# burn-research/OpenMEASURE

Hardware: AMD Instinct MI355X
Metric: SPR fit+reconstruct throughput (GB/s snapshot matrix) (higher is better)
Workload: dtype f64

## Files before the change

### openmeasure_amd/csrc/common.hpp

```cpp
#pragma once
#include <hip/hip_runtime.h>
#include <stdint.h>
#include <stdio.h>

#include "spr_hip.h"

typedef double f64x4 __attribute__((ext_vector_type(4)));
typedef double f64x2 __attribute__((ext_vector_type(2)));

void spr_set_error(const char *fmt, ...);

#define SPR_REQUIRE(cond, code, ...)      \
  do {                                    \
    if (!(cond)) {                        \
      spr_set_error(__VA_ARGS__);         \
      return (code);                      \
    }                                     \
  } while (0)

#define SPR_HIP_TRY(expr)                                                          \
  do {                                                                             \
    hipError_t e__ = (expr);                                                       \
    if (e__ != hipSuccess) {                                                       \
      spr_set_error("%s failed: %s (%s:%d)", #expr, hipGetErrorString(e__),       \
                    __FILE__, __LINE__);                                           \
      return SPR_E_HIP;                                                            \
    }                                                                              \
  } while (0)

#define SPR_LAUNCH_CHECK()                                                         \
  do {                                                                             \
    hipError_t e__ = hipGetLastError();                                            \
    if (e__ != hipSuccess) {                                                       \
      spr_set_error("kernel launch failed: %s (%s:%d)", hipGetErrorString(e__),   \
                    __FILE__, __LINE__);                                           \
      return SPR_E_HIP;                                                            \
    }                                                                              \
  } while (0)

int spr_cached_cus();

struct SegPlan {
  int64_t row0, n_rows, n_points;
  int32_t n_features;
  int32_t total_wg;
  int32_t chunk_rows;
};

__host__ __device__ inline void seg_range(const SegPlan &p, int f, int64_t &lo, int64_t &hi) {
  int64_t glo = (int64_t)f * p.n_points, ghi = glo + p.n_points;
  if (glo < p.row0) glo = p.row0;
  if (ghi > p.row0 + p.n_rows) ghi = p.row0 + p.n_rows;
  if (ghi < glo) ghi = glo;
  lo = glo - p.row0;
  hi = ghi - p.row0;
}

__host__ __device__ inline int seg_wgs(const SegPlan &p, int64_t rows) {
  if (rows <= 0) return 0;
  int64_t w = rows * (int64_t)p.total_wg / p.n_rows;
  int64_t chunks = (rows + p.chunk_rows - 1) / p.chunk_rows;
  if (w > chunks) w = chunks;
  if (w < 1) w = 1;
  return (int)w;
}

__host__ __device__ inline int seg_first_feature(const SegPlan &p) { return (int)(p.row0 / p.n_points); }
__host__ __device__ inline int seg_last_feature(const SegPlan &p) {
  int64_t f = (p.row0 + p.n_rows - 1) / p.n_points;
// ... 7 lines not shown
    int64_t lo, hi;
    seg_range(p, f, lo, hi);
    tot += seg_wgs(p, hi - lo);
  }
  return tot;
}

__device__ inline bool seg_locate(const SegPlan &p, int b, int &f, int &wl, int &wpf, int &base,
                                  int64_t &lo, int64_t &hi) {
  int acc = 0;
  int f1 = seg_last_feature(p);
  for (int ff = seg_first_feature(p); ff <= f1; ++ff) {
    seg_range(p, ff, lo, hi);
    int w = seg_wgs(p, hi - lo);
    if (b < acc + w) {
      f = ff; wl = b - acc; wpf = w; base = acc;
      return true;
    }
    acc += w;
  }
  return false;
}

template <int CTRL>
__device__ inline double dpp_f64(double v) {
  union { double d; int i[2]; } a, b;
  a.d = v;
  b.i[0] = __builtin_amdgcn_update_dpp(0, a.i[0], CTRL, 0xF, 0xF, true);
  b.i[1] = __builtin_amdgcn_update_dpp(0, a.i[1], CTRL, 0xF, 0xF, true);
  return b.d;
}

template <int WIDTH>
__device__ inline double group_sum_t(double v) {
  if (WIDTH >= 2) v += dpp_f64<0xB1>(v);
  if (WIDTH >= 4) v += dpp_f64<0x4E>(v);
  if (WIDTH >= 8) v += dpp_f64<0x141>(v);
  if (WIDTH >= 16) v += dpp_f64<0x140>(v);
  if (WIDTH >= 32) v += __shfl_xor(v, 16, 64);
  if (WIDTH >= 64) v += __shfl_xor(v, 32, 64);
  return v;
}

__device__ inline double group_sum(double v, int width) {
  for (int o = width >> 1; o > 0; o >>= 1) v += __shfl_xor(v, o, 64);
  return v;
// ... 16 lines not shown
```

### openmeasure_amd/csrc/project_ws.hip

```cpp
#include <type_traits>

#include "rowtile.hpp"

namespace {

#ifndef WS_ABLATE
#define WS_ABLATE 0
#endif
constexpr int WS_WAVES = 8;
constexpr int WS_ROWS = 16 * WS_WAVES;

template <int RT> struct WsLds { static constexpr int NC = 16 * RT, LDW = NC; static_assert(RT % 2 == 0, "column tiles come in pairs"); };

template <typename TX> struct WsPiece;
template <> struct WsPiece<double> { f64x2 a, b; };
template <> struct WsPiece<float> { float x, y, z, w; };

template <int VEC, typename TX>
__device__ inline WsPiece<TX> ws_load(const TX *__restrict__ rp, int col0, int m) {
  WsPiece<TX> p;
  if constexpr (std::is_same<TX, double>::value) {
    if (VEC) {
      p.a = *reinterpret_cast<const f64x2 *>(rp + col0);
      p.b = *reinterpret_cast<const f64x2 *>(rp + col0 + 2);
// ... 8 lines not shown
    } else {
      p.x = rp[col0 < m ? col0 : 0];         p.y = rp[col0 + 1 < m ? col0 + 1 : 0];
      p.z = rp[col0 + 2 < m ? col0 + 2 : 0]; p.w = rp[col0 + 3 < m ? col0 + 3 : 0];
    }
  }
  return p;
}

template <typename TX>
__device__ inline double ws_elem(const WsPiece<TX> &p, int t) {
  if constexpr (std::is_same<TX, double>::value) return t == 0 ? p.a.x : t == 1 ? p.a.y : t == 2 ? p.b.x : p.b.y;
  else return (double)(t == 0 ? p.x : t == 1 ? p.y : t == 2 ? p.z : p.w);
}

template <int MT, int RT, int VEC, typename TX, typename TU, bool NRM>
__global__ __launch_bounds__(WS_WAVES * 64) void project_ws_kernel(
    const TX *__restrict__ X, int64_t ldx, int m, int center_i, SegPlan plan, const double *__restrict__ inv_scale,
    const double *__restrict__ rowmean, const double *__restrict__ W, int r, TU *__restrict__ Ur, int64_t ldu,
    double *__restrict__ nrm2) {
  constexpr int K = 16 * MT, NJ = MT;
  constexpr int NC = WsLds<RT>::NC, LDW = WsLds<RT>::LDW;
  __shared__ double Wl[K * LDW];

  int f, wl, wpf, base;
  int64_t lo, hi;
  if (!seg_locate(plan, blockIdx.x, f, wl, wpf, base, lo, hi)) return;

  const int lane = threadIdx.x & 63;
  const int wave = __builtin_amdgcn_readfirstlane(threadIdx.x >> 6);
  const int li = lane & 15, kk = lane >> 4;
  const double isc = inv_scale[f];

  for (int e = threadIdx.x; e < K * NC; e += WS_WAVES * 64) {
    const int k = e / NC, c = e - k * NC;
    Wl[k * LDW + (c >> 5) * 32 + (c & 15) * 2 + ((c >> 4) & 1)] = (k < m && c < r) ? W[(int64_t)k * r + c] * isc : 0.0;
  }
  __syncthreads();
  double wbar[RT];
#pragma unroll
  for (int ct = 0; ct < RT; ++ct) {
    double sacc = 0.0;
    if (center_i != 0) {
      for (int k = kk; k < K; k += 4) sacc += Wl[k * LDW + (ct >> 1) * 32 + li * 2 + (ct & 1)];
      sacc += __shfl_xor(sacc, 16, 64);
      sacc += __shfl_xor(sacc, 32, 64);
    }
    wbar[ct] = sacc;
  }

  const int64_t nchunks = (hi - lo + WS_ROWS - 1) / WS_ROWS;
  int64_t c = wl;
  if (c >= nchunks) return;
  const double *wb = Wl + (4 * kk) * LDW + 2 * li;
  const double *wb_hi = wb + 128 * LDW;

  auto row_ptr = [&](int64_t cc) {
    int64_t row = lo + cc * WS_ROWS + 16 * wave + li;
    row = row < hi ? row : hi - 1;
    return X + row * ldx;
  };
  WsPiece<TX> areg[NJ];
  {
    const TX *rp = row_ptr(c);
#pragma unroll
    for (int j = 0; j < NJ; ++j) areg[j] = ws_load<VEC, TX>(rp, 16 * j + 4 * kk, m);
  }
  while (c < nchunks) {
    const int64_t cn = c + wpf;
    const TX *rpn = row_ptr(cn < nchunks ? cn : c);
    const int64_t blk0 = lo + c * WS_ROWS + 16 * wave;
    double mu[4];
#pragma unroll
    for (int i = 0; i < 4; ++i) {
      const int64_t rr = blk0 + kk + 4 * i;
      const double v = rowmean[rr < hi ? rr : hi - 1];
      mu[i] = center_i != 0 ? v : 0.0;
    }
    f64x4 acc[RT];
#pragma unroll
    for (int ct = 0; ct < RT; ++ct) acc[ct] = (f64x4){0.0, 0.0, 0.0, 0.0};
    f64x2 bcur[RT / 2], bnxt[RT / 2];
#pragma unroll
    for (int p = 0; p < RT / 2; ++p) bcur[p] = *reinterpret_cast<const f64x2 *>(wb + 32 * p);
#pragma unroll
    for (int j = 0; j < NJ; ++j) {
#pragma unroll
      for (int t = 0; t < 4; ++t) {
        const int sn = 4 * j + t + 1;
        const int jn = (sn >> 2) % NJ, tn = sn & 3;
        const double *wj = (jn < 8 ? wb : wb_hi) + (16 * (jn & 7) + tn) * LDW;
#pragma unroll
        for (int p = 0; p < RT / 2; ++p) bnxt[p] = *reinterpret_cast<const f64x2 *>(wj + 32 * p);
        const double a = ws_elem<TX>(areg[j], t);
#pragma unroll
        for (int p = 0; p < RT / 2; ++p) {
#if WS_ABLATE == 1
          asm volatile("" ::"v"(a), "v"(bcur[p].x), "v"(bcur[p].y));
#else
          acc[2 * p] = __builtin_amdgcn_mfma_f64_16x16x4f64(a, bcur[p].x, acc[2 * p], 0, 0, 0);
          acc[2 * p + 1] = __builtin_amdgcn_mfma_f64_16x16x4f64(a, bcur[p].y, acc[2 * p + 1], 0, 0, 0);
#endif
        }
        if (t == 3) areg[j] = ws_load<VEC, TX>(rpn, 16 * j + 4 * kk, m);
        __builtin_amdgcn_sched_group_barrier(0x100, RT / 2, 0);
        __builtin_amdgcn_sched_group_barrier(0x008, RT, 0);
        __builtin_amdgcn_sched_barrier(0);
#pragma unroll
        for (int p = 0; p < RT / 2; ++p) bcur[p] = bnxt[p];
      }
    }
    {
      const bool full = (blk0 + 16 <= hi) && (r == NC);
      TU *up = Ur + (blk0 + kk) * ldu + li;
      double q[4] = {0.0, 0.0, 0.0, 0.0};
#pragma unroll
      for (int ct = 0; ct < RT; ++ct) {
        const double s[4] = {acc[ct].x - mu[0] * wbar[ct], acc[ct].y - mu[1] * wbar[ct],
                             acc[ct].z - mu[2] * wbar[ct], acc[ct].w - mu[3] * wbar[ct]};
        if (NRM) {
#pragma unroll
          for (int i = 0; i < 4; ++i) { const double v = (double)(TU)s[i]; q[i] = fma(v, v, q[i]); }
        }
        if (full) {
#pragma unroll
          for (int i = 0; i < 4; ++i) up[4 * i * ldu + 16 * ct] = (TU)s[i];
        } else if (16 * ct + li < r) {
#pragma unroll
          for (int i = 0; i < 4; ++i)
            if (blk0 + kk + 4 * i < hi) up[4 * i * ldu + 16 * ct] = (TU)s[i];
        }
      }
      if (NRM) {
#pragma unroll
        for (int i = 0; i < 4; ++i) {
          const double t = group_sum_t<16>(q[i]);
          if (li == i && blk0 + kk + 4 * i < hi) nrm2[blk0 + kk + 4 * i] = t;
        }
      }
    }
    c = cn;
  }
}

template <int MT, int RT, typename TX, typename TU>
int ws_launch(const TX *X, int64_t n_rows, int32_t m, int64_t ldx, int64_t row0, int64_t n_points, int32_t n_features,
              int center, const double *inv_scale, const double *rowmean, const double *W, int32_t r, TU *Ur,
              int64_t ldu, int accumulate, double *nrm2, hipStream_t st) {
  const int cus = spr_cached_cus();
  SegPlan plan;
  plan.row0 = row0; plan.n_rows = n_rows; plan.n_points = n_points; plan.n_features = n_features;
  static const int narrow_per_cu = [] { const char *e = getenv("SPR_WS_WG_PER_CU"); const int v = e ? atoi(e) : 2; return v >= 1 && v <= 4 ? v : 2; }();
  plan.total_wg = (cus > 0 ? cus : 256) * (MT <= 4 ? narrow_per_cu : 1);
  plan.chunk_rows = WS_ROWS;
  const int grid = seg_total_wgs(plan);
  const bool vec = (m == 16 * MT) && ((sizeof(TX) * ldx) % 16 == 0) && ((reinterpret_cast<uintptr_t>(X) & 15) == 0);
  if (!vec) return SPR_E_UNSUPPORTED;
  if (nrm2)
    hipLaunchKernelGGL((project_ws_kernel<MT, RT, 1, TX, TU, true>), dim3(grid), dim3(WS_WAVES * 64), 0, st, X, ldx, (int)m,
                       center, plan, inv_scale, rowmean, W, (int)r, Ur, ldu, nrm2);
  else
    hipLaunchKernelGGL((project_ws_kernel<MT, RT, 1, TX, TU, false>), dim3(grid), dim3(WS_WAVES * 64), 0, st, X, ldx, (int)m,
                       center, plan, inv_scale, rowmean, W, (int)r, Ur, ldu, nrm2);
  SPR_LAUNCH_CHECK();
  return SPR_OK;
}

}

#include "project_ws.hpp"

template <typename TX, typename TU>
int spr_project_ws(const TX *d_X, int64_t n_rows, int32_t m, int64_t ldx, int64_t row0, int64_t n_points,
                   int32_t n_features, int32_t center, const double *d_inv_scale, const double *d_rowmean,
                   const double *d_W, int32_t r, TU *d_Ur, int64_t ldu, int32_t accumulate, double *d_rownorm2,
                   hipStream_t st) {
  if (accumulate) return SPR_E_UNSUPPORTED;
  const int mt = spr_round_mt(m);
// ... 27 lines not shown
```

### openmeasure_amd/csrc/runtime.hip

```cpp
#include <stdarg.h>
#include <stdlib.h>
#include <string.h>

#include "common.hpp"

namespace {
thread_local char g_err[512] = "";
}

void spr_set_error(const char *fmt, ...) {
  va_list ap;
  va_start(ap, fmt);
  vsnprintf(g_err, sizeof(g_err), fmt, ap);
  va_end(ap);
}

int spr_cached_cus() {
  static int cus = 0;
  if (cus) return cus;
  int dev = 0;
  hipDeviceProp_t prop;
  if (hipGetDevice(&dev) != hipSuccess || hipGetDeviceProperties(&prop, dev) != hipSuccess) return 0;
  cus = prop.multiProcessorCount;
  if (const char *e = getenv("SPR_RESERVE_CUS")) {
    const int k = atoi(e);
    if (k > 0 && k < cus) cus -= k;
  }
  return cus;
}

extern "C" int spr_abi_version(void) { return SPR_ABI_VERSION; }

extern "C" const char *spr_last_error(void) { return g_err; }

extern "C" int spr_device_cus(int *out_cus) {
  SPR_REQUIRE(out_cus != nullptr, SPR_E_INVALID, "spr_device_cus: NULL output");
  const int c = spr_cached_cus();
  SPR_REQUIRE(c > 0, SPR_E_HIP, "spr_device_cus: no HIP device");
  *out_cus = c;
  return SPR_OK;
}

namespace {
__global__ __launch_bounds__(256) void upload_kernel(const uint64_t *__restrict__ src, uint64_t *__restrict__ dst,
                                                     int64_t n_words) {
  for (int64_t i = (int64_t)blockIdx.x * 256 + threadIdx.x; i < n_words; i += (int64_t)gridDim.x * 256)
    dst[i] = __builtin_nontemporal_load(src + i);
}
}

extern "C" int spr_upload_bytes(void *d_dst, const void *h_pinned_src, int64_t n_bytes, void *stream) {
// ... 38 lines not shown
```

### openmeasure_amd/csrc/stats_gram.hip

```cpp
#include <stdlib.h>

#include <type_traits>

#include "rowtile.hpp"

#ifndef GRAM_UNIT_PAIRING
#define GRAM_UNIT_PAIRING 1
#endif
#ifndef GRAM_ABLATE
#define GRAM_ABLATE 0
#endif
#if GRAM_ABLATE == 1
#define GRAM_MFMA(a, b, c) ({ asm volatile("" ::"v"(a), "v"(b)); (c); })
#else
#define GRAM_MFMA(a, b, c) __builtin_amdgcn_mfma_f64_16x16x4f64((a), (b), (c), 0, 0, 0)
#endif

namespace {

template <int MT>
struct GramShape {
  static constexpr int MPAD = 16 * MT;
  static constexpr int MP = MPAD + ((MT % 2 == 0) ? 16 : 0);
  static constexpr int T = MT * (MT + 1) / 2;
// ... 11 lines not shown
template <> struct GramCfg<4>  { static constexpr int NW = 8,  R = GRAM4_R, KS = 4; static constexpr bool DBUF = true; static constexpr int LPRMAX = GRAM4_LPR; };
template <> struct GramCfg<6>  { static constexpr int NW = 12, R = 48, KS = 4; static constexpr bool DBUF = true; static constexpr int LPRMAX = 16; };
template <> struct GramCfg<8>  { static constexpr int NW = 8,  R = 32, KS = 2; static constexpr bool DBUF = true; static constexpr int LPRMAX = 16; };
template <> struct GramCfg<12> { static constexpr int NW = 12, R = 24, KS = 2; static constexpr bool DBUF = false; static constexpr int LPRMAX = 32; };
#ifndef GRAM_DBUF16
#define GRAM_DBUF16 false
#endif
template <> struct GramCfg<16> { static constexpr int NW = 8,  R = 32, KS = 1; static constexpr bool DBUF = GRAM_DBUF16; static constexpr int LPRMAX = 16; };

template <int MT> struct GramOut { static constexpr int KSO = (GramCfg<MT>::KS >= 4) ? 1 : GramCfg<MT>::KS; };

constexpr int tri_index(int mt, int ti, int tj) { return ti * mt - ti * (ti - 1) / 2 + (tj - ti); }

template <int MT>
__device__ inline void tile_coords(int idx, int &ti, int &tj) {
  ti = 0;
  while (ti < MT - 1 && idx >= MT - ti) { idx -= MT - ti; ++ti; }
  tj = ti + idx;
  if (tj > MT - 1) tj = MT - 1;
}

template <int MT, int U, int VEC, typename TX>
__device__ inline void gram_wave(const TX *__restrict__ X, int64_t ldx, int m, int center,
                                 int64_t lo, int64_t hi, int wl, int wpf, int ks, int wave, int lane,
                                 double *__restrict__ lds0, double *__restrict__ lds1,
                                 double *__restrict__ rowmean, double *__restrict__ stat_part,
                                 double *__restrict__ slab, double *__restrict__ rowsum) {
  using S = GramShape<MT>;
  using C = GramCfg<MT>;
  constexpr int R = C::R, KS = C::KS, NW = C::NW, MP = S::MP, T = S::T;
  constexpr int KROWS = R / KS, KSTEPS = KROWS / 4;
  constexpr int RA = U, RB = MT - 1 - U;
  constexpr int NA = MT - RA;
  constexpr int NB = (RB != RA) ? MT - RB : 0;
  static_assert(KROWS % 4 == 0, "k slice must be a multiple of the MFMA depth");
  using RT = RowTile<MT, R, MP, NW, C::LPRMAX, TX>;

  f64x4 accA[NA];
  f64x4 accB[NB > 0 ? NB : 1];
#pragma unroll
  for (int j = 0; j < NA; ++j) accA[j] = (f64x4){0.0, 0.0, 0.0, 0.0};
#pragma unroll
  for (int j = 0; j < NB; ++j) accB[j] = (f64x4){0.0, 0.0, 0.0, 0.0};

  RowStats st;
  st.init();
  RT tile;
// ... 80 lines not shown
        }
#pragma unroll
        for (int j = 0; j < NB; ++j) {
          double *tp = red + tri_index(MT, RB, RB + j) * 256;
          tp[0] = accB[j].x; tp[64] = accB[j].y; tp[128] = accB[j].z; tp[192] = accB[j].w;
        }
      }
      __syncthreads();
      if (ks == s - 1) {
#pragma unroll
        for (int j = 0; j < NA; ++j) {
          const double *tp = red + tri_index(MT, RA, RA + j) * 256;
          accA[j].x += tp[0]; accA[j].y += tp[64]; accA[j].z += tp[128]; accA[j].w += tp[192];
        }
#pragma unroll
        for (int j = 0; j < NB; ++j) {
          const double *tp = red + tri_index(MT, RB, RB + j) * 256;
          accB[j].x += tp[0]; accB[j].y += tp[64]; accB[j].z += tp[128]; accB[j].w += tp[192];
        }
      }
    }
  }
  if (KSO == KS || ks == 0) {
    double *sp = slab + ((int64_t)blockIdx.x * KSO + (KSO == KS ? ks : 0)) * T * 256 + lane;
#pragma unroll
    for (int j = 0; j < NA; ++j) {
      double *tp = sp + (int64_t)tri_index(MT, RA, RA + j) * 256;
      tp[0] = accA[j].x; tp[64] = accA[j].y; tp[128] = accA[j].z; tp[192] = accA[j].w;
    }
#pragma unroll
    for (int j = 0; j < NB; ++j) {
      double *tp = sp + (int64_t)tri_index(MT, RB, RB + j) * 256;
      tp[0] = accB[j].x; tp[64] = accB[j].y; tp[128] = accB[j].z; tp[192] = accB[j].w;
    }
  }
  if ((lane % RT::LPR) == 0) {
    double *q = stat_part + ((int64_t)blockIdx.x * RT::ROWS_PER_IT + wave * RT::RPW + lane / RT::LPR) * 3;
    q[0] = st.cnt; q[1] = st.mean(); q[2] = st.m2();
  }
}

__device__ inline void chan_merge(double &n, double &mu, double &m2, double nb, double mb, double sb) {
  if (nb > 0.0) {
    const double tot = n + nb, d = mb - mu;
    mu += d * nb / tot;
    m2 += sb + d * d * n * nb / tot;
    n = tot;
  }
}

template <int MT, int U, typename TX, bool EXT, bool SUMS>
__device__ inline void gram_wave_own(const TX *__restrict__ X, int64_t ldx, int64_t lo, int64_t hi, int wl, int wpf, int ks,
                                     int wave, int lane, double *__restrict__ lds0, double *__restrict__ lds1,
                                     double *__restrict__ rowmean, double *__restrict__ slab, double *__restrict__ rowsum) {
  using S = GramShape<MT>;
  using C = GramCfg<MT>;
  constexpr int R = C::R, KS = C::KS, NW = C::NW, MP = S::MP, T = S::T;
  constexpr int KROWS = R / KS, KSTEPS = KROWS / 4;
  constexpr int RA = U, RB = MT - 1 - U;
  constexpr int NA = MT - RA;
  constexpr int NB = (RB != RA) ? MT - RB : 0;
  using RT = RowTile<MT, R, MP, NW, C::LPRMAX, TX>;

  f64x4 accA[NA];
  f64x4 accB[NB > 0 ? NB : 1];
#pragma unroll
  for (int j = 0; j < NA; ++j) accA[j] = (f64x4){0.0, 0.0, 0.0, 0.0};
#pragma unroll
  for (int j = 0; j < NB; ++j) accB[j] = (f64x4){0.0, 0.0, 0.0, 0.0};

  RT tile;
  const int64_t nchunks = (hi - lo + R - 1) / R;
  const int64_t lane_off = (int64_t)(wave * RT::RPW + lane / RT::LPR) * ldx;
  auto base_of = [&](int64_t row0) { return X + row0 * ldx; };
  int64_t c = wl;
// ... 45 lines not shown
        for (int j = 0; j < NA; ++j) accA[j] = GRAM_MFMA(op[k & 1][0], op[k & 1][j], accA[j]);
#pragma unroll
        for (int j = 0; j < NB; ++j) accB[j] = GRAM_MFMA(op[k & 1][RB - RA], op[k & 1][RB - RA + j], accB[j]);
        if (nfull) stage(std::true_type{}, k); else stage(std::false_type{}, k);
      }
    } else {
#pragma unroll
      for (int k = 0; k < KSTEPS; ++k) {
        double op[NA];
#pragma unroll
        for (int j = 0; j < NA; ++j) op[j] = p[k * 4 * MP + 16 * j];
#pragma unroll
        for (int j = 0; j < NA; ++j) accA[j] = GRAM_MFMA(op[0], op[j], accA[j]);
#pragma unroll
        for (int j = 0; j < NB; ++j) accB[j] = GRAM_MFMA(op[RB - RA], op[RB - RA + j], accB[j]);
        if (nfull) stage(std::true_type{}, k); else stage(std::false_type{}, k);
      }
    }
    buf ^= 1;
    c = cn;
    cn = c2;
    nrow0 = n2row0;
  }
  double *sp = slab + ((int64_t)blockIdx.x * KS + ks) * T * 256 + lane;
#pragma unroll
  for (int j = 0; j < NA; ++j) {
    double *tp = sp + (int64_t)tri_index(MT, RA, RA + j) * 256;
    tp[0] = accA[j].x; tp[64] = accA[j].y; tp[128] = accA[j].z; tp[192] = accA[j].w;
  }
#pragma unroll
  for (int j = 0; j < NB; ++j) {
    double *tp = sp + (int64_t)tri_index(MT, RB, RB + j) * 256;
    tp[0] = accB[j].x; tp[64] = accB[j].y; tp[128] = accB[j].z; tp[192] = accB[j].w;
  }
}

template <int MT, typename TX, bool EXT, bool SUMS>
__global__ __launch_bounds__(GramCfg<MT>::NW * 64) void stats_gram_own_kernel(
    const TX *__restrict__ X, int64_t ldx, SegPlan plan, double *__restrict__ rowmean, double *__restrict__ slab,
    double *__restrict__ rowsum) {
  using S = GramShape<MT>;
  using C = GramCfg<MT>;
  constexpr int NU = S::NU;
  __shared__ double lds[2][C::R * S::MP];
  int f, wl, wpf, base;
  int64_t lo, hi;
  if (!seg_locate(plan, blockIdx.x, f, wl, wpf, base, lo, hi)) return;
  const int lane = threadIdx.x & 63;
  const int wave = __builtin_amdgcn_readfirstlane(threadIdx.x >> 6);
  const int ks = wave / NU;
  const int unit = (GRAM_UNIT_PAIRING && NU == 8 && C::KS == 1) ? ((wave < 4) ? wave : 11 - wave) : wave % NU;
#define GRAM_UNIT(UV)                                                                                          \
  case UV:                                                                                                     \
    if constexpr (UV < NU)                                                                                     \
      gram_wave_own<MT, UV, TX, EXT, SUMS>(X, ldx, lo, hi, wl, wpf, ks, wave, lane, lds[0], lds[1], rowmean, slab, rowsum); \
    break;
  switch (unit) {
    GRAM_UNIT(0) GRAM_UNIT(1) GRAM_UNIT(2) GRAM_UNIT(3) GRAM_UNIT(4) GRAM_UNIT(5) GRAM_UNIT(6) GRAM_UNIT(7)
    default: break;
  }
#undef GRAM_UNIT
}

constexpr int RS_THREADS = 1024;
__global__ __launch_bounds__(RS_THREADS) void gram_rowmean_stats_kernel(const double *__restrict__ rowmean, SegPlan plan,
                                                                        int slots_per_wg, double *__restrict__ stat_part) {
  __shared__ double sn[RS_THREADS / 64], smu[RS_THREADS / 64], sm2[RS_THREADS / 64];
  int f, wl, wpf, base;
  int64_t lo, hi;
  if (!seg_locate(plan, blockIdx.x, f, wl, wpf, base, lo, hi)) return;
  const int lane = threadIdx.x & 63, wave = threadIdx.x >> 6;
  RowStats st;
  st.init();
  const int64_t step = (int64_t)wpf * RS_THREADS;
  int64_t row = lo + (int64_t)wl * RS_THREADS + threadIdx.x;
  for (; row + 3 * step < hi; row += 4 * step) {
    const double a = rowmean[row], b = rowmean[row + step], c = rowmean[row + 2 * step], d = rowmean[row + 3 * step];
    st.push(a, true); st.push(b, true); st.push(c, true); st.push(d, true);
  }
  for (; row < hi; row += step) st.push(rowmean[row], true);
  double n = st.cnt, mu = st.mean(), m2 = st.m2();
  for (int o = 32; o > 0; o >>= 1) {
    const double on = __shfl_down(n, o, 64), om = __shfl_down(mu, o, 64), os = __shfl_down(m2, o, 64);
    chan_merge(n, mu, m2, on, om, os);
  }
  if (lane == 0) { sn[wave] = n; smu[wave] = mu; sm2[wave] = m2; }
  __syncthreads();
  double *q = stat_part + (int64_t)blockIdx.x * slots_per_wg * 3;
  if (threadIdx.x == 0) {
    n = 0.0; mu = 0.0; m2 = 0.0;
    for (int w = 0; w < RS_THREADS / 64; ++w) chan_merge(n, mu, m2, sn[w], smu[w], sm2[w]);
    q[0] = n; q[1] = mu; q[2] = m2;
  }
  for (int e = 3 + threadIdx.x; e < slots_per_wg * 3; e += RS_THREADS) q[e] = 0.0;
}

template <int MT, int VEC, typename TX>
__global__ __launch_bounds__(GramCfg<MT>::NW * 64) void stats_gram_kernel(
    const TX *__restrict__ X, int64_t ldx, int m, int center_i, SegPlan plan,
    double *__restrict__ rowmean, double *__restrict__ stat_part, double *__restrict__ slab, double *__restrict__ rowsum) {
  using S = GramShape<MT>;
  using C = GramCfg<MT>;
  constexpr int NU = S::NU;
  static_assert(NU * C::KS == C::NW, "waves = units x k slices");
  __shared__ double lds[2][C::R * S::MP];

  int f, wl, wpf, base;
  int64_t lo, hi;
  if (!seg_locate(plan, blockIdx.x, f, wl, wpf, base, lo, hi)) return;

  const int lane = threadIdx.x & 63;
  const int wave = __builtin_amdgcn_readfirstlane(threadIdx.x >> 6);
  const int unit = wave % NU, ks = wave / NU;
#define GRAM_UNIT(UV)                                                                                        \
  case UV:                                                                                                   \
    if constexpr (UV < NU)                                                                                   \
      gram_wave<MT, UV, VEC, TX>(X, ldx, m, center_i, lo, hi, wl, wpf, ks, wave, lane, lds[0],    \
                        lds[1], rowmean, stat_part, slab, rowsum);                                           \
    break;
  switch (unit) {
    GRAM_UNIT(0) GRAM_UNIT(1) GRAM_UNIT(2) GRAM_UNIT(3) GRAM_UNIT(4) GRAM_UNIT(5) GRAM_UNIT(6) GRAM_UNIT(7)
    default: break;
  }
#undef GRAM_UNIT
}

template <int MT>
__global__ __launch_bounds__(1024) void gram_finalize_kernel(
    const double *__restrict__ slab, const double *__restrict__ stat_part, int m, SegPlan plan,
    int slots_per_wg, double *__restrict__ gram, double *__restrict__ fstats, int ldg, int origin) {
  constexpr int T = GramShape<MT>::T;
  constexpr int KS = GramOut<MT>::KSO;
  __shared__ double red[4][256];
  const int f = blockIdx.y;
  const int tile = blockIdx.x;
  int base = 0, wpf = 0;
  {
    int acc = 0;
    const int f0 = seg_first_feature(plan), f1 = seg_last_feature(plan);
    for (int ff = f0; ff <= f1; ++ff) {
      int64_t lo, hi;
      seg_range(plan, ff, lo, hi);
      const int w = seg_wgs(plan, hi - lo);
      if (ff == f) { base = acc; wpf = w; }
      acc += w;
    }
  }
  int ti, tj;
  tile_coords<MT>(tile, ti, tj);
  const int e = threadIdx.x & 255, g = threadIdx.x >> 8;
  const int np = wpf * KS;
  const double *sp = slab + ((int64_t)base * KS * T + tile) * 256 + e;
  const int64_t stride = (int64_t)T * 256;
  double s0 = 0.0, s1 = 0.0, s2 = 0.0, s3 = 0.0;
  int p = g;
  for (; p + 12 < np; p += 16) {
    s0 += sp[p * stride];
    s1 += sp[(p + 4) * stride];
    s2 += sp[(p + 8) * stride];
    s3 += sp[(p + 12) * stride];
  }
  for (; p < np; p += 4) s0 += sp[p * stride];
  red[g][e] = (s0 + s1) + (s2 + s3);
  __syncthreads();
  if (g == 0) {
    const double sum = (red[0][e] + red[1][e]) + (red[2][e] + red[3][e]);
    const int l = e & 63, reg = e >> 6;
    const int gi = ti * 16 + (l >> 4) + 4 * reg, gj = tj * 16 + (l & 15);
    if (gi < m && gj < m) {
      double *G = gram + (int64_t)f * ldg * ldg + (int64_t)origin * ldg + origin;
// ... 23 lines not shown
  }
}

template <int MT>
int occupancy_wgs() {
  static int cached = 0;
  if (cached) return cached;
  int per_cu = 0;
  if (hipOccupancyMaxActiveBlocksPerMultiprocessor(&per_cu, stats_gram_kernel<MT, 2, double>, GramCfg<MT>::NW * 64, 0) != hipSuccess ||
      per_cu < 1)
    per_cu = 1;
  if (per_cu > 4) per_cu = 4;
  const int cus = spr_cached_cus();
  cached = per_cu * (cus > 0 ? cus : 256);
  return cached;
}

template <int MT>
SegPlan make_plan(int64_t n_rows, int64_t row0, int64_t n_points, int32_t n_features) {
  SegPlan p;
  p.row0 = row0; p.n_rows = n_rows; p.n_points = n_points; p.n_features = n_features;
  p.total_wg = occupancy_wgs<MT>();
  p.chunk_rows = GramCfg<MT>::R;
  return p;
}

template <int MT>
size_t workspace_bytes(int32_t n_features) {
  using RT = RowTile<MT, GramCfg<MT>::R, GramShape<MT>::MP, GramCfg<MT>::NW, GramCfg<MT>::LPRMAX>;
  const int64_t max_grid = (int64_t)occupancy_wgs<MT>() + n_features;
  return (size_t)max_grid * GramCfg<MT>::KS * GramShape<MT>::T * 256 * sizeof(double) +
         (size_t)max_grid * RT::ROWS_PER_IT * 3 * sizeof(double);
}

template <int MT, typename TX>
int launch(const TX *X, int64_t n_rows, int32_t m, int64_t ldx, int64_t row0, int64_t n_points,
           int32_t n_features, int center, double *rowmean, void *ws, size_t ws_bytes, hipStream_t st,
           double *rowsum = nullptr) {
  SPR_REQUIRE(ws_bytes >= workspace_bytes<MT>(n_features), SPR_E_WORKSPACE,
              "spr_stats_gram_f64: workspace %zu < %zu", ws_bytes, workspace_bytes<MT>(n_features));
  SPR_REQUIRE(!rowsum || center == 2, SPR_E_INVALID, "spr_stats_gram: row sums are an output of centre mode 2 only");
  SegPlan plan = make_plan<MT>(n_rows, row0, n_points, n_features);
  const int grid = seg_total_wgs(plan);
  const int64_t max_grid = (int64_t)occupancy_wgs<MT>() + n_features;
  SPR_REQUIRE(grid >= 1 && grid <= max_grid, SPR_E_INVALID, "spr_stats_gram_f64: bad grid %d", grid);
  double *slab = static_cast<double *>(ws);
  double *stat_part = slab + (size_t)max_grid * GramCfg<MT>::KS * GramShape<MT>::T * 256;
  const int vec_ok = (m % 2 == 0) && (ldx % 2 == 0) && ((reinterpret_cast<uintptr_t>(X) & (2 * sizeof(TX) - 1)) == 0);
  const int lm = vec_ok ? ((m == 16 * MT) ? 2 : 1) : 0;
#define SG_LAUNCH(LM)                                                                                         \
  hipLaunchKernelGGL((stats_gram_kernel<MT, LM, TX>), dim3(grid), dim3(GramCfg<MT>::NW * 64), 0, st, X, ldx, (int)m, \
                     center, plan, rowmean, stat_part, slab, rowsum)
  using RTL = RowTile<MT, GramCfg<MT>::R, GramShape<MT>::MP, GramCfg<MT>::NW, GramCfg<MT>::LPRMAX, TX>;
  static const bool own_on = [] { const char *e = getenv("SPR_GRAM_OWN"); return !(e && e[0] == '0'); }();
  if (MT >= 8 && lm == 2 && (center == 1 || center == 2) && own_on && (sizeof(TX) * ldx) % 16 == 0 &&
      (reinterpret_cast<uintptr_t>(X) & 15) == 0) {
    if constexpr (MT >= 8) {
      if (center == 1)
        hipLaunchKernelGGL((stats_gram_own_kernel<MT, TX, false, false>), dim3(grid), dim3(GramCfg<MT>::NW * 64), 0, st, X, ldx,
                           plan, rowmean, slab, rowsum);
      else if (!rowsum)
        hipLaunchKernelGGL((stats_gram_own_kernel<MT, TX, true, false>), dim3(grid), dim3(GramCfg<MT>::NW * 64), 0, st, X, ldx,
                           plan, rowmean, slab, rowsum);
      else
        hipLaunchKernelGGL((stats_gram_own_kernel<MT, TX, true, true>), dim3(grid), dim3(GramCfg<MT>::NW * 64), 0, st, X, ldx,
                           plan, rowmean, slab, rowsum);
// ... 147 lines not shown
```

Baseline: 1173.

## Balance row chunks evenly across workgroups independent of feature boundaries

Adds a balanced segment plan that splits all rows into equal contiguous chunk ranges per workgroup, so one workgroup may cover pieces of several features. Kernels loop over those pieces and write partials to per-piece slots, and the reduction maps each feature to its slot range. This targets load imbalance and tail effects from sizing workgroups per feature. In exchange there are extra syncs and W reloads when a workgroup crosses a feature boundary, and the slot indexing becomes more complex.

After: 1180 (median of 6 runs). No clear change (+0.6%).

```diff
diff --git a/openmeasure_amd/csrc/common.hpp b/openmeasure_amd/csrc/common.hpp
--- a/openmeasure_amd/csrc/common.hpp
+++ b/openmeasure_amd/csrc/common.hpp
@@ -45,6 +45,7 @@
   int32_t n_features;
   int32_t total_wg;
   int32_t chunk_rows;
+  int32_t balanced = 0;
 };
 
 __host__ __device__ inline void seg_range(const SegPlan &p, int f, int64_t &lo, int64_t &hi) {
@@ -98,6 +99,81 @@
   return false;
 }
 
+__host__ __device__ inline int64_t bal_chunks(const SegPlan &p) { return (p.n_rows + p.chunk_rows - 1) / p.chunk_rows; }
+__host__ __device__ inline int bal_wgs(const SegPlan &p) {
+  const int64_t n = bal_chunks(p);
+  return (int)(n < p.total_wg ? n : p.total_wg);
+}
+__host__ __device__ inline void bal_share(const SegPlan &p, int b, int64_t &lo, int64_t &hi) {
+  const int64_t n = bal_chunks(p), w = bal_wgs(p);
+  lo = (int64_t)b * n / w * p.chunk_rows;
+  hi = (int64_t)(b + 1) * n / w * p.chunk_rows;
+  if (lo > p.n_rows) lo = p.n_rows;
+  if (hi > p.n_rows) hi = p.n_rows;
+}
+__host__ __device__ inline int bal_owner(const SegPlan &p, int64_t row) {
+  const int64_t n = bal_chunks(p), w = bal_wgs(p), c = row / p.chunk_rows;
+  return (int)(((c + 1) * w - 1) / n);
+}
+__host__ __device__ inline int seg_feature_of(const SegPlan &p, int64_t row) { return (int)((p.row0 + row) / p.n_points); }
+
+inline int seg_grid(const SegPlan &p) { return p.balanced ? bal_wgs(p) : seg_total_wgs(p); }
+
+struct SegPiece {
+  int f, wl, wpf, slot;
+  int64_t lo, hi;
+};
+
+__host__ __device__ inline bool seg_piece(const SegPlan &p, int b, int k, SegPiece &pc) {
+  if (!p.balanced) {
+    if (k > 0) return false;
+    int acc = 0;
+    const int f1 = seg_last_feature(p);
+    for (int ff = seg_first_feature(p); ff <= f1; ++ff) {
+      seg_range(p, ff, pc.lo, pc.hi);
+      const int w = seg_wgs(p, pc.hi - pc.lo);
+      if (b < acc + w) {
+        pc.f = ff; pc.wl = b - acc; pc.wpf = w; pc.slot = b;
+        return true;
+      }
+      acc += w;
+    }
+    return false;
+  }
+  int64_t slo, shi;
+  bal_share(p, b, slo, shi);
+  if (slo >= shi) return false;
+  const int f = seg_feature_of(p, slo) + k;
+  if (f > seg_feature_of(p, shi - 1)) return false;
+  seg_range(p, f, pc.lo, pc.hi);
+  if (pc.lo < slo) pc.lo = slo;
+  if (pc.hi > shi) pc.hi = shi;
+  pc.f = f; pc.wl = 0; pc.wpf = 1; pc.slot = b + f - seg_first_feature(p);
+  return true;
+}
+
+__host__ __device__ inline void seg_feature_slots(const SegPlan &p, int f, int &s0, int &ns) {
+  s0 = 0; ns = 0;
+  if (f < seg_first_feature(p) || f > seg_last_feature(p)) return;
+  int64_t lo, hi;
+  seg_range(p, f, lo, hi);
+  if (hi <= lo) return;
+  if (p.balanced) {
+    const int b0 = bal_owner(p, lo), b1 = bal_owner(p, hi - 1);
+    s0 = b0 + f - seg_first_feature(p);
+    ns = b1 - b0 + 1;
+    return;
+  }
+  for (int ff = seg_first_feature(p); ff < f; ++ff) {
+    int64_t l, h;
+    seg_range(p, ff, l, h);
+    s0 += seg_wgs(p, h - l);
+  }
+  ns = seg_wgs(p, hi - lo);
+}
+
+bool spr_seg_balance();
+
 template <int CTRL>
 __device__ inline double dpp_f64(double v) {
   union { double d; int i[2]; } a, b;
diff --git a/openmeasure_amd/csrc/project_ws.hip b/openmeasure_amd/csrc/project_ws.hip
--- a/openmeasure_amd/csrc/project_ws.hip
+++ b/openmeasure_amd/csrc/project_ws.hip
@@ -54,123 +54,125 @@
   constexpr int NC = WsLds<RT>::NC, LDW = WsLds<RT>::LDW;
   __shared__ double Wl[K * LDW];
 
-  int f, wl, wpf, base;
-  int64_t lo, hi;
-  if (!seg_locate(plan, blockIdx.x, f, wl, wpf, base, lo, hi)) return;
-
   const int lane = threadIdx.x & 63;
   const int wave = __builtin_amdgcn_readfirstlane(threadIdx.x >> 6);
   const int li = lane & 15, kk = lane >> 4;
-  const double isc = inv_scale[f];
-
-  for (int e = threadIdx.x; e < K * NC; e += WS_WAVES * 64) {
-    const int k = e / NC, c = e - k * NC;
-    Wl[k * LDW + (c >> 5) * 32 + (c & 15) * 2 + ((c >> 4) & 1)] = (k < m && c < r) ? W[(int64_t)k * r + c] * isc : 0.0;
-  }
-  __syncthreads();
-  double wbar[RT];
-#pragma unroll
-  for (int ct = 0; ct < RT; ++ct) {
-    double sacc = 0.0;
-    if (center_i != 0) {
-      for (int k = kk; k < K; k += 4) sacc += Wl[k * LDW + (ct >> 1) * 32 + li * 2 + (ct & 1)];
-      sacc += __shfl_xor(sacc, 16, 64);
-      sacc += __shfl_xor(sacc, 32, 64);
-    }
-    wbar[ct] = sacc;
-  }
-
-  const int64_t nchunks = (hi - lo + WS_ROWS - 1) / WS_ROWS;
-  int64_t c = wl;
-  if (c >= nchunks) return;
-  const double *wb = Wl + (4 * kk) * LDW + 2 * li;
-  const double *wb_hi = wb + 128 * LDW;
-
-  auto row_ptr = [&](int64_t cc) {
-    int64_t row = lo + cc * WS_ROWS + 16 * wave + li;
-    row = row < hi ? row : hi - 1;
-    return X + row * ldx;
-  };
-  WsPiece<TX> areg[NJ];
-  {
-    const TX *rp = row_ptr(c);
-#pragma unroll
-    for (int j = 0; j < NJ; ++j) areg[j] = ws_load<VEC, TX>(rp, 16 * j + 4 * kk, m);
-  }
-  while (c < nchunks) {
-    const int64_t cn = c + wpf;
-    const TX *rpn = row_ptr(cn < nchunks ? cn : c);
-    const int64_t blk0 = lo + c * WS_ROWS + 16 * wave;
-    double mu[4];
-#pragma unroll
-    for (int i = 0; i < 4; ++i) {
-      const int64_t rr = blk0 + kk + 4 * i;
-      const double v = rowmean[rr < hi ? rr : hi - 1];
-      mu[i] = center_i != 0 ? v : 0.0;
-    }
-    f64x4 acc[RT];
-#pragma unroll
-    for (int ct = 0; ct < RT; ++ct) acc[ct] = (f64x4){0.0, 0.0, 0.0, 0.0};
-    f64x2 bcur[RT / 2], bnxt[RT / 2];
-#pragma unroll
-    for (int p = 0; p < RT / 2; ++p) bcur[p] = *reinterpret_cast<const f64x2 *>(wb + 32 * p);
-#pragma unroll
-    for (int j = 0; j < NJ; ++j) {
-#pragma unroll
-      for (int t = 0; t < 4; ++t) {
-        const int sn = 4 * j + t + 1;
-        const int jn = (sn >> 2) % NJ, tn = sn & 3;
-        const double *wj = (jn < 8 ? wb : wb_hi) + (16 * (jn & 7) + tn) * LDW;
-#pragma unroll
-        for (int p = 0; p < RT / 2; ++p) bnxt[p] = *reinterpret_cast<const f64x2 *>(wj + 32 * p);
-        const double a = ws_elem<TX>(areg[j], t);
-#pragma unroll
-        for (int p = 0; p < RT / 2; ++p) {
-#if WS_ABLATE == 1
-          asm volatile("" ::"v"(a), "v"(bcur[p].x), "v"(bcur[p].y));
-#else
-          acc[2 * p] = __builtin_amdgcn_mfma_f64_16x16x4f64(a, bcur[p].x, acc[2 * p], 0, 0, 0);
-          acc[2 * p + 1] = __builtin_amdgcn_mfma_f64_16x16x4f64(a, bcur[p].y, acc[2 * p + 1], 0, 0, 0);
-#endif
+  SegPiece pc;
+  for (int piece = 0; seg_piece(plan, blockIdx.x, piece, pc); ++piece) {
+    if (piece > 0) __syncthreads();
+    const int64_t lo = pc.lo, hi = pc.hi;
+    const int wl = pc.wl, wpf = pc.wpf;
+    const double isc = inv_scale[pc.f];
+
+    for (int e = threadIdx.x; e < K * NC; e += WS_WAVES * 64) {
+      const int k = e / NC, c = e - k * NC;
+      Wl[k * LDW + (c >> 5) * 32 + (c & 15) * 2 + ((c >> 4) & 1)] = (k < m && c < r) ? W[(int64_t)k * r + c] * isc : 0.0;
+    }
+    __syncthreads();
+    double wbar[RT];
+#pragma unroll
+    for (int ct = 0; ct < RT; ++ct) {
+      double sacc = 0.0;
+      if (center_i != 0) {
+        for (int k = kk; k < K; k += 4) sacc += Wl[k * LDW + (ct >> 1) * 32 + li * 2 + (ct & 1)];
+        sacc += __shfl_xor(sacc, 16, 64);
+        sacc += __shfl_xor(sacc, 32, 64);
+      }
+      wbar[ct] = sacc;
+    }
+
+    const int64_t nchunks = (hi - lo + WS_ROWS - 1) / WS_ROWS;
+    int64_t c = wl;
+    if (c >= nchunks) continue;
+    const double *wb = Wl + (4 * kk) * LDW + 2 * li;
+    const double *wb_hi = wb + 128 * LDW;
+
+    auto row_ptr = [&](int64_t cc) {
+      int64_t row = lo + cc * WS_ROWS + 16 * wave + li;
+      row = row < hi ? row : hi - 1;
+      return X + row * ldx;
+    };
+    WsPiece<TX> areg[NJ];
+    {
+      const TX *rp = row_ptr(c);
+#pragma unroll
+      for (int j = 0; j < NJ; ++j) areg[j] = ws_load<VEC, TX>(rp, 16 * j + 4 * kk, m);
+    }
+    while (c < nchunks) {
+      const int64_t cn = c + wpf;
+      const TX *rpn = row_ptr(cn < nchunks ? cn : c);
+      const int64_t blk0 = lo + c * WS_ROWS + 16 * wave;
+      double mu[4];
+#pragma unroll
+      for (int i = 0; i < 4; ++i) {
+        const int64_t rr = blk0 + kk + 4 * i;
+        const double v = rowmean[rr < hi ? rr : hi - 1];
+        mu[i] = center_i != 0 ? v : 0.0;
+      }
+      f64x4 acc[RT];
+#pragma unroll
+      for (int ct = 0; ct < RT; ++ct) acc[ct] = (f64x4){0.0, 0.0, 0.0, 0.0};
+      f64x2 bcur[RT / 2], bnxt[RT / 2];
+#pragma unroll
+      for (int p = 0; p < RT / 2; ++p) bcur[p] = *reinterpret_cast<const f64x2 *>(wb + 32 * p);
+#pragma unroll
+      for (int j = 0; j < NJ; ++j) {
+#pragma unroll
+        for (int t = 0; t < 4; ++t) {
+          const int sn = 4 * j + t + 1;
+          const int jn = (sn >> 2) % NJ, tn = sn & 3;
+          const double *wj = (jn < 8 ? wb : wb_hi) + (16 * (jn & 7) + tn) * LDW;
+#pragma unroll
+          for (int p = 0; p < RT / 2; ++p) bnxt[p] = *reinterpret_cast<const f64x2 *>(wj + 32 * p);
+          const double a = ws_elem<TX>(areg[j], t);
+#pragma unroll
+          for (int p = 0; p < RT / 2; ++p) {
+  #if WS_ABLATE == 1
+            asm volatile("" ::"v"(a), "v"(bcur[p].x), "v"(bcur[p].y));
+  #else
+            acc[2 * p] = __builtin_amdgcn_mfma_f64_16x16x4f64(a, bcur[p].x, acc[2 * p], 0, 0, 0);
+            acc[2 * p + 1] = __builtin_amdgcn_mfma_f64_16x16x4f64(a, bcur[p].y, acc[2 * p + 1], 0, 0, 0);
+  #endif
+          }
+          if (t == 3) areg[j] = ws_load<VEC, TX>(rpn, 16 * j + 4 * kk, m);
+          __builtin_amdgcn_sched_group_barrier(0x100, RT / 2, 0);
+          __builtin_amdgcn_sched_group_barrier(0x008, RT, 0);
+          __builtin_amdgcn_sched_barrier(0);
+#pragma unroll
+          for (int p = 0; p < RT / 2; ++p) bcur[p] = bnxt[p];
         }
-        if (t == 3) areg[j] = ws_load<VEC, TX>(rpn, 16 * j + 4 * kk, m);
-        __builtin_amdgcn_sched_group_barrier(0x100, RT / 2, 0);
-        __builtin_amdgcn_sched_group_barrier(0x008, RT, 0);
-        __builtin_amdgcn_sched_barrier(0);
-#pragma unroll
-        for (int p = 0; p < RT / 2; ++p) bcur[p] = bnxt[p];
-      }
-    }
-    {
-      const bool full = (blk0 + 16 <= hi) && (r == NC);
-      TU *up = Ur + (blk0 + kk) * ldu + li;
-      double q[4] = {0.0, 0.0, 0.0, 0.0};
-#pragma unroll
-      for (int ct = 0; ct < RT; ++ct) {
-        const double s[4] = {acc[ct].x - mu[0] * wbar[ct], acc[ct].y - mu[1] * wbar[ct],
-                             acc[ct].z - mu[2] * wbar[ct], acc[ct].w - mu[3] * wbar[ct]};
+      }
+      {
+        const bool full = (blk0 + 16 <= hi) && (r == NC);
+        TU *up = Ur + (blk0 + kk) * ldu + li;
+        double q[4] = {0.0, 0.0, 0.0, 0.0};
+#pragma unroll
+        for (int ct = 0; ct < RT; ++ct) {
+          const double s[4] = {acc[ct].x - mu[0] * wbar[ct], acc[ct].y - mu[1] * wbar[ct],
+                               acc[ct].z - mu[2] * wbar[ct], acc[ct].w - mu[3] * wbar[ct]};
+          if (NRM) {
+#pragma unroll
+            for (int i = 0; i < 4; ++i) { const double v = (double)(TU)s[i]; q[i] = fma(v, v, q[i]); }
+          }
+          if (full) {
+#pragma unroll
+            for (int i = 0; i < 4; ++i) up[4 * i * ldu + 16 * ct] = (TU)s[i];
+          } else if (16 * ct + li < r) {
+#pragma unroll
+            for (int i = 0; i < 4; ++i)
+              if (blk0 + kk + 4 * i < hi) up[4 * i * ldu + 16 * ct] = (TU)s[i];
+          }
+        }
         if (NRM) {
 #pragma unroll
-          for (int i = 0; i < 4; ++i) { const double v = (double)(TU)s[i]; q[i] = fma(v, v, q[i]); }
+          for (int i = 0; i < 4; ++i) {
+            const double t = group_sum_t<16>(q[i]);
+            if (li == i && blk0 + kk + 4 * i < hi) nrm2[blk0 + kk + 4 * i] = t;
+          }
         }
-        if (full) {
-#pragma unroll
-          for (int i = 0; i < 4; ++i) up[4 * i * ldu + 16 * ct] = (TU)s[i];
-        } else if (16 * ct + li < r) {
-#pragma unroll
-          for (int i = 0; i < 4; ++i)
-            if (blk0 + kk + 4 * i < hi) up[4 * i * ldu + 16 * ct] = (TU)s[i];
-        }
-      }
-      if (NRM) {
-#pragma unroll
-        for (int i = 0; i < 4; ++i) {
-          const double t = group_sum_t<16>(q[i]);
-          if (li == i && blk0 + kk + 4 * i < hi) nrm2[blk0 + kk + 4 * i] = t;
-        }
-      }
-    }
-    c = cn;
+      }
+      c = cn;
+    }
   }
 }
 
@@ -184,7 +186,8 @@
   static const int narrow_per_cu = [] { const char *e = getenv("SPR_WS_WG_PER_CU"); const int v = e ? atoi(e) : 2; return v >= 1 && v <= 4 ? v : 2; }();
   plan.total_wg = (cus > 0 ? cus : 256) * (MT <= 4 ? narrow_per_cu : 1);
   plan.chunk_rows = WS_ROWS;
-  const int grid = seg_total_wgs(plan);
+  plan.balanced = spr_seg_balance();
+  const int grid = seg_grid(plan);
   const bool vec = (m == 16 * MT) && ((sizeof(TX) * ldx) % 16 == 0) && ((reinterpret_cast<uintptr_t>(X) & 15) == 0);
   if (!vec) return SPR_E_UNSUPPORTED;
   if (nrm2)
diff --git a/openmeasure_amd/csrc/runtime.hip b/openmeasure_amd/csrc/runtime.hip
--- a/openmeasure_amd/csrc/runtime.hip
+++ b/openmeasure_amd/csrc/runtime.hip
@@ -27,6 +27,11 @@
     if (k > 0 && k < cus) cus -= k;
   }
   return cus;
+}
+
+bool spr_seg_balance() {
+  static const bool on = [] { const char *e = getenv("SPR_SEG_BALANCE"); return !(e && e[0] == '0'); }();
+  return on;
 }
 
 extern "C" int spr_abi_version(void) { return SPR_ABI_VERSION; }
diff --git a/openmeasure_amd/csrc/stats_gram.hip b/openmeasure_amd/csrc/stats_gram.hip
--- a/openmeasure_amd/csrc/stats_gram.hip
+++ b/openmeasure_amd/csrc/stats_gram.hip
@@ -57,7 +57,7 @@
 
 template <int MT, int U, int VEC, typename TX>
 __device__ inline void gram_wave(const TX *__restrict__ X, int64_t ldx, int m, int center,
-                                 int64_t lo, int64_t hi, int wl, int wpf, int ks, int wave, int lane,
+                                 int64_t lo, int64_t hi, int wl, int wpf, int slot, int ks, int wave, int lane,
                                  double *__restrict__ lds0, double *__restrict__ lds1,
                                  double *__restrict__ rowmean, double *__restrict__ stat_part,
                                  double *__restrict__ slab, double *__restrict__ rowsum) {
@@ -184,7 +184,7 @@
     }
   }
   if (KSO == KS || ks == 0) {
-    double *sp = slab + ((int64_t)blockIdx.x * KSO + (KSO == KS ? ks : 0)) * T * 256 + lane;
+    double *sp = slab + ((int64_t)slot * KSO + (KSO == KS ? ks : 0)) * T * 256 + lane;
 #pragma unroll
     for (int j = 0; j < NA; ++j) {
       double *tp = sp + (int64_t)tri_index(MT, RA, RA + j) * 256;
@@ -197,7 +197,7 @@
     }
   }
   if ((lane % RT::LPR) == 0) {
-    double *q = stat_part + ((int64_t)blockIdx.x * RT::ROWS_PER_IT + wave * RT::RPW + lane / RT::LPR) * 3;
+    double *q = stat_part + ((int64_t)slot * RT::ROWS_PER_IT + wave * RT::RPW + lane / RT::LPR) * 3;
     q[0] = st.cnt; q[1] = st.mean(); q[2] = st.m2();
   }
 }
@@ -212,7 +212,7 @@
 }
 
 template <int MT, int U, typename TX, bool EXT, bool SUMS>
-__device__ inline void gram_wave_own(const TX *__restrict__ X, int64_t ldx, int64_t lo, int64_t hi, int wl, int wpf, int ks,
+__device__ inline void gram_wave_own(const TX *__restrict__ X, int64_t ldx, int64_t lo, int64_t hi, int wl, int wpf, int slot, int ks,
                                      int wave, int lane, double *__restrict__ lds0, double *__restrict__ lds1,
                                      double *__restrict__ rowmean, double *__restrict__ slab, double *__restrict__ rowsum) {
   using S = GramShape<MT>;
@@ -304,7 +304,7 @@
     cn = c2;
     nrow0 = n2row0;
   }
-  double *sp = slab + ((int64_t)blockIdx.x * KS + ks) * T * 256 + lane;
+  double *sp = slab + ((int64_t)slot * KS + ks) * T * 256 + lane;
 #pragma unroll
   for (int j = 0; j < NA; ++j) {
     double *tp = sp + (int64_t)tri_index(MT, RA, RA + j) * 256;
@@ -325,56 +325,61 @@
   using C = GramCfg<MT>;
   constexpr int NU = S::NU;
   __shared__ double lds[2][C::R * S::MP];
-  int f, wl, wpf, base;
-  int64_t lo, hi;
-  if (!seg_locate(plan, blockIdx.x, f, wl, wpf, base, lo, hi)) return;
   const int lane = threadIdx.x & 63;
   const int wave = __builtin_amdgcn_readfirstlane(threadIdx.x >> 6);
   const int ks = wave / NU;
   const int unit = (GRAM_UNIT_PAIRING && NU == 8 && C::KS == 1) ? ((wave < 4) ? wave : 11 - wave) : wave % NU;
+  SegPiece pc;
+  for (int piece = 0; seg_piece(plan, blockIdx.x, piece, pc); ++piece) {
+    if (piece > 0) __syncthreads();
 #define GRAM_UNIT(UV)                                                                                          \
   case UV:                                                                                                     \
     if constexpr (UV < NU)                                                                                     \
-      gram_wave_own<MT, UV, TX, EXT, SUMS>(X, ldx, lo, hi, wl, wpf, ks, wave, lane, lds[0], lds[1], rowmean, slab, rowsum); \
+      gram_wave_own<MT, UV, TX, EXT, SUMS>(X, ldx, pc.lo, pc.hi, pc.wl, pc.wpf, pc.slot, ks, wave, lane, lds[0], lds[1], \
+                                           rowmean, slab, rowsum);                                             \
     break;
-  switch (unit) {
-    GRAM_UNIT(0) GRAM_UNIT(1) GRAM_UNIT(2) GRAM_UNIT(3) GRAM_UNIT(4) GRAM_UNIT(5) GRAM_UNIT(6) GRAM_UNIT(7)
-    default: break;
-  }
+    switch (unit) {
+      GRAM_UNIT(0) GRAM_UNIT(1) GRAM_UNIT(2) GRAM_UNIT(3) GRAM_UNIT(4) GRAM_UNIT(5) GRAM_UNIT(6) GRAM_UNIT(7)
+      default: break;
+    }
 #undef GRAM_UNIT
+  }
 }
 
 constexpr int RS_THREADS = 1024;
 __global__ __launch_bounds__(RS_THREADS) void gram_rowmean_stats_kernel(const double *__restrict__ rowmean, SegPlan plan,
                                                                         int slots_per_wg, double *__restrict__ stat_part) {
   __shared__ double sn[RS_THREADS / 64], smu[RS_THREADS / 64], sm2[RS_THREADS / 64];
-  int f, wl, wpf, base;
-  int64_t lo, hi;
-  if (!seg_locate(plan, blockIdx.x, f, wl, wpf, base, lo, hi)) return;
   const int lane = threadIdx.x & 63, wave = threadIdx.x >> 6;
-  RowStats st;
-  st.init();
-  const int64_t step = (int64_t)wpf * RS_THREADS;
-  int64_t row = lo + (int64_t)wl * RS_THREADS + threadIdx.x;
-  for (; row + 3 * step < hi; row += 4 * step) {
-    const double a = rowmean[row], b = rowmean[row + step], c = rowmean[row + 2 * step], d = rowmean[row + 3 * step];
-    st.push(a, true); st.push(b, true); st.push(c, true); st.push(d, true);
-  }
-  for (; row < hi; row += step) st.push(rowmean[row], true);
-  double n = st.cnt, mu = st.mean(), m2 = st.m2();
-  for (int o = 32; o > 0; o >>= 1) {
-    const double on = __shfl_down(n, o, 64), om = __shfl_down(mu, o, 64), os = __shfl_down(m2, o, 64);
-    chan_merge(n, mu, m2, on, om, os);
-  }
-  if (lane == 0) { sn[wave] = n; smu[wave] = mu; sm2[wave] = m2; }
-  __syncthreads();
-  double *q = stat_part + (int64_t)blockIdx.x * slots_per_wg * 3;
-  if (threadIdx.x == 0) {
-    n = 0.0; mu = 0.0; m2 = 0.0;
-    for (int w = 0; w < RS_THREADS / 64; ++w) chan_merge(n, mu, m2, sn[w], smu[w], sm2[w]);
-    q[0] = n; q[1] = mu; q[2] = m2;
-  }
-  for (int e = 3 + threadIdx.x; e < slots_per_wg * 3; e += RS_THREADS) q[e] = 0.0;
+  SegPiece pc;
+  for (int piece = 0; seg_piece(plan, blockIdx.x, piece, pc); ++piece) {
+    if (piece > 0) __syncthreads();
+    const int64_t lo = pc.lo, hi = pc.hi;
+    const int wl = pc.wl, wpf = pc.wpf;
+    RowStats st;
+    st.init();
+    const int64_t step = (int64_t)wpf * RS_THREADS;
+    int64_t row = lo + (int64_t)wl * RS_THREADS + threadIdx.x;
+    for (; row + 3 * step < hi; row += 4 * step) {
+      const double a = rowmean[row], b = rowmean[row + step], c = rowmean[row + 2 * step], d = rowmean[row + 3 * step];
+      st.push(a, true); st.push(b, true); st.push(c, true); st.push(d, true);
+    }
+    for (; row < hi; row += step) st.push(rowmean[row], true);
+    double n = st.cnt, mu = st.mean(), m2 = st.m2();
+    for (int o = 32; o > 0; o >>= 1) {
+      const double on = __shfl_down(n, o, 64), om = __shfl_down(mu, o, 64), os = __shfl_down(m2, o, 64);
+      chan_merge(n, mu, m2, on, om, os);
+    }
+    if (lane == 0) { sn[wave] = n; smu[wave] = mu; sm2[wave] = m2; }
+    __syncthreads();
+    double *q = stat_part + (int64_t)pc.slot * slots_per_wg * 3;
+    if (threadIdx.x == 0) {
+      n = 0.0; mu = 0.0; m2 = 0.0;
+      for (int w = 0; w < RS_THREADS / 64; ++w) chan_merge(n, mu, m2, sn[w], smu[w], sm2[w]);
+      q[0] = n; q[1] = mu; q[2] = m2;
+    }
+    for (int e = 3 + threadIdx.x; e < slots_per_wg * 3; e += RS_THREADS) q[e] = 0.0;
+  }
 }
 
 template <int MT, int VEC, typename TX>
@@ -387,24 +392,24 @@
   static_assert(NU * C::KS == C::NW, "waves = units x k slices");
   __shared__ double lds[2][C::R * S::MP];
 
-  int f, wl, wpf, base;
-  int64_t lo, hi;
-  if (!seg_locate(plan, blockIdx.x, f, wl, wpf, base, lo, hi)) return;
-
   const int lane = threadIdx.x & 63;
   const int wave = __builtin_amdgcn_readfirstlane(threadIdx.x >> 6);
   const int unit = wave % NU, ks = wave / NU;
+  SegPiece pc;
+  for (int piece = 0; seg_piece(plan, blockIdx.x, piece, pc); ++piece) {
+    if (piece > 0) __syncthreads();
 #define GRAM_UNIT(UV)                                                                                        \
   case UV:                                                                                                   \
     if constexpr (UV < NU)                                                                                   \
-      gram_wave<MT, UV, VEC, TX>(X, ldx, m, center_i, lo, hi, wl, wpf, ks, wave, lane, lds[0],    \
+      gram_wave<MT, UV, VEC, TX>(X, ldx, m, center_i, pc.lo, pc.hi, pc.wl, pc.wpf, pc.slot, ks, wave, lane, lds[0], \
                         lds[1], rowmean, stat_part, slab, rowsum);                                           \
     break;
-  switch (unit) {
-    GRAM_UNIT(0) GRAM_UNIT(1) GRAM_UNIT(2) GRAM_UNIT(3) GRAM_UNIT(4) GRAM_UNIT(5) GRAM_UNIT(6) GRAM_UNIT(7)
-    default: break;
-  }
+    switch (unit) {
+      GRAM_UNIT(0) GRAM_UNIT(1) GRAM_UNIT(2) GRAM_UNIT(3) GRAM_UNIT(4) GRAM_UNIT(5) GRAM_UNIT(6) GRAM_UNIT(7)
+      default: break;
+    }
 #undef GRAM_UNIT
+  }
 }
 
 template <int MT>
@@ -416,18 +421,8 @@
   __shared__ double red[4][256];
   const int f = blockIdx.y;
   const int tile = blockIdx.x;
-  int base = 0, wpf = 0;
-  {
-    int acc = 0;
-    const int f0 = seg_first_feature(plan), f1 = seg_last_feature(plan);
-    for (int ff = f0; ff <= f1; ++ff) {
-      int64_t lo, hi;
-      seg_range(plan, ff, lo, hi);
-      const int w = seg_wgs(plan, hi - lo);
-      if (ff == f) { base = acc; wpf = w; }
-      acc += w;
-    }
-  }
+  int base, wpf;
+  seg_feature_slots(plan, f, base, wpf);
   int ti, tj;
   tile_coords<MT>(tile, ti, tj);
   const int e = threadIdx.x & 255, g = threadIdx.x >> 8;
@@ -497,6 +492,7 @@
   p.row0 = row0; p.n_rows = n_rows; p.n_points = n_points; p.n_features = n_features;
   p.total_wg = occupancy_wgs<MT>();
   p.chunk_rows = GramCfg<MT>::R;
+  p.balanced = spr_seg_balance();
   return p;
 }
 
@@ -516,7 +512,7 @@
               "spr_stats_gram_f64: workspace %zu < %zu", ws_bytes, workspace_bytes<MT>(n_features));
   SPR_REQUIRE(!rowsum || center == 2, SPR_E_INVALID, "spr_stats_gram: row sums are an output of centre mode 2 only");
   SegPlan plan = make_plan<MT>(n_rows, row0, n_points, n_features);
-  const int grid = seg_total_wgs(plan);
+  const int grid = seg_grid(plan);
   const int64_t max_grid = (int64_t)occupancy_wgs<MT>() + n_features;
   SPR_REQUIRE(grid >= 1 && grid <= max_grid, SPR_E_INVALID, "spr_stats_gram_f64: bad grid %d", grid);
   double *slab = static_cast<double *>(ws);
```
